# calebhabesh/NM03-Capstone-Project

Hardware: AMD Instinct MI355X
Metric: DICOM slices/sec through full pipeline (T1+C cohort) at 1/2/4/8 MI355X (higher is better)
Workload: dtype fp32

## Files before the change

include/nm03/cohort.h:

```cpp
#pragma once

#include <cstdint>
#include <memory>
#include <string>
#include <vector>

namespace nm03::cohort {

int extract_file_number(const std::string& filename);

std::string default_data_root();
std::string with_slash(const std::string& p);
std::string cohort_dir(const std::string& data_root);
std::string test_slice_path(const std::string& data_root);

std::vector<std::string> find_patient_dirs(const std::string& cohort_root);

struct Series {
  std::string series_dir;
  std::vector<std::string> files;
};
Series list_patient_series(const std::string& cohort_root, const std::string& patient_id);

void setup_output_dir(const std::string& dir);
void setup_output_dirs(const std::vector<std::string>& dirs, int threads);
void make_dirs(const std::string& dir);

class OutputReaper {
 public:
  explicit OutputReaper(int threads = 4);
  ~OutputReaper();
  OutputReaper(const OutputReaper&) = delete;
  OutputReaper& operator=(const OutputReaper&) = delete;
  void wipe(const std::string& dir);
  void wipe(const std::vector<std::string>& dirs);
  void drain();
  int64_t files_reaped() const;

  struct Impl;

 private:
  std::unique_ptr<Impl> impl_;
};

std::string stem(const std::string& path);
std::string filename(const std::string& path);

}
```

include/nm03/dicom.h:

```cpp
#pragma once

#include <cstdint>
#include <memory>
#include <string>
#include <vector>

#include "nm03/common.h"

namespace nm03::dicom {

enum class Syntax : uint8_t {
  kImplicitLE,
  kExplicitLE,
  kExplicitBE,
  kDeflatedLE,
  kRleLossless,
  kJpegLossless,
  kJpegBaseline,
  kJpegExtended,
};

const char* syntax_name(Syntax s);

struct Header {
// ... 10 lines not shown
  double slice_thickness = 0;
  double spacing_between_slices = 0;
  std::string photometric, transfer_syntax, sop_instance_uid, series_uid, patient_id, modality;
  Syntax syntax = Syntax::kExplicitLE;
  size_t pixel_offset = 0;
  size_t pixel_length = 0;
  bool invert = false;
  std::shared_ptr<const std::vector<uint8_t>> decoded;
  size_t frame_bytes() const { return (size_t)rows * cols * (bits_allocated / 8); }
  bool native_le() const { return decoded || syntax != Syntax::kExplicitBE; }
  const uint8_t* pixel_base(const uint8_t* file) const { return decoded ? decoded->data() : file; }
};

Header parse(const uint8_t* data, size_t size);

Header parse_prefix(const uint8_t* data, size_t avail, size_t size);

void copy_pixels16(const Header& h, const uint8_t* data, size_t size, uint16_t* dst, int frame = 0);

int select_frame(const Header& h, int policy);

void invert_samples(uint16_t* px, size_t n, int bits);

std::vector<uint8_t> read_file(const std::string& path);
size_t read_file_into(const std::string& path, std::vector<uint8_t>& buf);

enum class ReadMode { kDirect, kStaged, kMapped };

class SliceFile {
 public:
  explicit SliceFile(const std::string& path, ReadMode mode = ReadMode::kDirect, size_t prefix = 16384);
  SliceFile(int dirfd, const char* name, const std::string& path, ReadMode mode = ReadMode::kDirect,
            size_t prefix = 16384);
  ~SliceFile();
  SliceFile(const SliceFile&) = delete;
  SliceFile& operator=(const SliceFile&) = delete;
  size_t size() const { return size_; }
  void map_at(void* addr, size_t cap) {
    map_at_ = addr;
    map_cap_ = cap;
  }
  const Header& header(std::vector<uint8_t>& buf);
  void pixels16(uint16_t* dst, int frame = 0);
  bool direct() const { return !whole_; }
  const uint16_t* staged_samples(int frame = 0) const;

 private:
  void pread_all(void* dst, size_t n, size_t off);
  void stat_size();
  bool size_known_ = false;
  const uint8_t* data() const { return map_ ? map_ : buf_->data(); }
  std::string path_;
  const uint8_t* map_ = nullptr;
  bool own_map_ = true;
  void* map_at_ = nullptr;
  size_t map_cap_ = 0;
  int fd_ = -1;
  size_t size_ = 0;
  ReadMode mode_ = ReadMode::kDirect;
  size_t prefix_ = 16384;
  size_t have_ = 0;
  Header h_;
  bool whole_ = true;
  std::vector<uint8_t>* buf_ = nullptr;
};

void stream_copy(void* dst, const void* src, size_t n);
void stream_copy_unfenced(void* dst, const void* src, size_t n);

struct WriteSpec {
  int rows = 256, cols = 256;
  PixelType type = kU16;
  int bits_stored = 16;
  const uint16_t* pixels = nullptr;
  bool write_rescale = false;
  float slope = 1.f, intercept = 0.f;
  float spacing_x = 1.f, spacing_y = 1.f;
  double slice_thickness = 1.0;
  double spacing_between_slices = 0;
  int instance_number = 1;
  double position[3] = {0, 0, 0};
  bool write_position = true;
  std::string patient_id = "PGBM-000";
  std::string study_uid = "1.2.826.0.1.3680043.10.1", series_uid = "1.2.826.0.1.3680043.10.2",
              sop_uid = "1.2.826.0.1.3680043.10.3";
// ... 13 lines not shown
```

include/nm03/jpeg.h:

```cpp
#pragma once

#include <atomic>
#include <cstdint>
#include <string>
#include <vector>

#include "nm03/jpeg_common.h"

namespace nm03::jpeg {

struct Tables {
  int quality = 75;
  uint16_t qluma[64];
  uint16_t qchroma[64];
  int32_t div_luma[64];
  int32_t div_chroma[64];
};

Tables make_tables(int quality);

std::vector<uint8_t> make_header(int width, int height, const Tables& t, Sampling s = kSampling420);

std::vector<uint8_t> encode_gray(const uint8_t* gray, int width, int height, int stride, int quality,
                                 Sampling s = kSampling420);

std::vector<uint8_t> encode_scan_gray(const uint8_t* gray, int width, int height, int stride, const Tables& t,
                                      Sampling s = kSampling420);

std::vector<uint8_t> encode_rgb(const uint8_t* rgb, int width, int height, int stride, int quality,
                                Sampling s = kSampling420);
std::vector<uint8_t> encode_scan_rgb(const uint8_t* rgb, int width, int height, int stride, const Tables& t,
                                     Sampling s = kSampling420);

void write_jpeg_file(const std::string& path, const std::vector<uint8_t>& header, const uint8_t* scan,
                     size_t scan_len);
void write_jpeg_at(int dirfd, const std::string& dir, const std::string& name, const std::vector<uint8_t>& header,
                   const uint8_t* scan, size_t scan_len,
                   std::atomic<uint8_t>* creating = nullptr);
void write_bytes_at(int dirfd, const std::string& dir, const std::string& name, const void* data, size_t len,
                    std::atomic<uint8_t>* creating = nullptr);

}
```

src/io/cohort.cpp:

```cpp
#include "nm03/cohort.h"

#include <dirent.h>
#include <fcntl.h>
#include <linux/capability.h>
#include <pthread.h>
#include <signal.h>
#include <sys/stat.h>
#include <sys/syscall.h>
#include <unistd.h>

#include <algorithm>
#include <atomic>
#include <cerrno>
#include <condition_variable>
#include <deque>
#include <mutex>
#include <set>
#include <thread>
#include <cstdlib>
#include <cstring>
#include <filesystem>
#include <stdexcept>
#include <system_error>

// ... 244 lines not shown
void OutputReaper::wipe(const std::string& dir_in) {
  std::string dir = dir_in;
  while (dir.size() > 1 && dir.back() == '/') dir.pop_back();
  const size_t slash = dir.rfind('/');
  const std::string parent = slash == std::string::npos ? "." : slash == 0 ? "/" : dir.substr(0, slash);
  make_dirs(parent);
  impl_->sweep_parent(parent);
  const std::string trash = parent + "/" + kTrashPrefix + std::to_string(::getpid()) + "-" +
                            std::to_string(impl_->seq.fetch_add(1));
  if (::rename(dir.c_str(), trash.c_str()) == 0) {
    impl_->push(trash);
  } else if (errno != ENOENT) {
    setup_output_dir(dir);
    return;
  }
  if (::mkdir(dir.c_str(), 0755) != 0 && errno != EEXIST)
    throw std::runtime_error("Failed to setup output directory: " + dir + " (" + std::strerror(errno) + ")");
}

void OutputReaper::wipe(const std::vector<std::string>& dirs) {
  for (const auto& d : dirs) wipe(d);
}

void OutputReaper::drain() {
  std::unique_lock<std::mutex> g(impl_->m);
  impl_->idle_cv.wait(g, [&] { return impl_->q.empty() && impl_->busy == 0; });
}

int64_t OutputReaper::files_reaped() const { return impl_->files.load(); }

std::string stem(const std::string& path) { return fs::path(path).stem().string(); }
std::string filename(const std::string& path) { return fs::path(path).filename().string(); }

}
```

src/io/dicom.cpp:

```cpp
#include "nm03/dicom.h"
#include "nm03/jpeg_dct.h"
#include "nm03/jpeg_lossless.h"

#include <fcntl.h>
#include <immintrin.h>
#include <sys/mman.h>
#include <sys/stat.h>
#include <unistd.h>
#include <zlib.h>

#include <algorithm>
#include <cerrno>
#include <cstdio>
#include <cstdlib>
#include <cstring>
#include <fstream>

namespace nm03::dicom {
namespace {

constexpr uint32_t kUndefined = 0xFFFFFFFFu;

struct Cursor {
  const uint8_t* d;
// ... 518 lines not shown
    std::memcpy(dst, src, n * 2);
  }
  if (h.invert) invert_samples(dst, n, h.bits_stored);
}

size_t read_file_into(const std::string& path, std::vector<uint8_t>& buf) {
  int fd = ::open(path.c_str(), O_RDONLY | O_CLOEXEC);
  if (fd < 0) throw SliceError("Cannot open file: " + path + " (" + std::strerror(errno) + ")");
  struct stat st;
  if (fstat(fd, &st) != 0) {
    ::close(fd);
    throw SliceError("Cannot stat file: " + path);
  }
  size_t n = (size_t)st.st_size;
  if (buf.size() < n) buf.resize(n);
  size_t got = 0;
  while (got < n) {
    ssize_t r = ::read(fd, buf.data() + got, n - got);
    if (r < 0 && errno == EINTR) continue;
    if (r <= 0) {
      ::close(fd);
      throw SliceError("Read error on file: " + path);
    }
    got += (size_t)r;
  }
  ::close(fd);
  return n;
}

SliceFile::SliceFile(const std::string& path, ReadMode mode, size_t prefix)
    : SliceFile(AT_FDCWD, path.c_str(), path, mode, prefix) {}

SliceFile::SliceFile(int dirfd, const char* name, const std::string& path, ReadMode mode, size_t prefix)
    : path_(path), mode_(mode), prefix_(prefix < 1024 ? 1024 : prefix) {
  fd_ = ::openat(dirfd, name, O_RDONLY | O_CLOEXEC);
  if (fd_ < 0) throw SliceError("Cannot open file: " + path + " (" + std::strerror(errno) + ")");
  if (mode_ == ReadMode::kStaged) return;
  stat_size();
}

void SliceFile::stat_size() {
  struct stat st;
  if (fstat(fd_, &st) != 0) {
    ::close(fd_);
    fd_ = -1;
    throw SliceError("Cannot stat file: " + path_);
  }
  size_ = (size_t)st.st_size;
  size_known_ = true;
}

SliceFile::~SliceFile() {
  if (map_ && own_map_) ::munmap(const_cast<uint8_t*>(map_), size_);
  if (fd_ >= 0) ::close(fd_);
}

void SliceFile::pread_all(void* dst, size_t n, size_t off) {
  size_t got = 0;
  while (got < n) {
    ssize_t r = ::pread(fd_, (uint8_t*)dst + got, n - got, (off_t)(off + got));
    if (r < 0 && errno == EINTR) continue;
    if (r <= 0) throw SliceError("Read error on file: " + path_);
    got += (size_t)r;
  }
}

const Header& SliceFile::header(std::vector<uint8_t>& buf) {
  buf_ = &buf;
  if (mode_ == ReadMode::kStaged && !size_known_) {
    if (buf.size() < (256u << 10)) buf.resize(256u << 10);
    size_t got = 0;
    for (;;) {
      const ssize_t r = ::pread(fd_, buf.data() + got, buf.size() - got, (off_t)got);
      if (r < 0 && errno == EINTR) continue;
      if (r < 0) throw SliceError("Read error on file: " + path_);
      got += (size_t)r;
      if (got < buf.size() || r == 0) break;
      stat_size();
      if (size_ <= got) break;
      buf.resize(size_);
    }
    size_ = got;
    size_known_ = true;
    have_ = size_;
    try {
      h_ = parse(buf.data(), size_);
    } catch (const SliceError&) {
      stat_size();
      if (size_ <= got) throw;
      if (buf.size() < size_) buf.resize(size_);
      pread_all(buf.data() + got, size_ - got, got);
      have_ = size_;
      h_ = parse(buf.data(), size_);
    }
    whole_ = true;
    return h_;
  }
  if (mode_ == ReadMode::kMapped && size_ > 0) {
    const bool fixed = map_at_ && size_ <= map_cap_;
    void* m = ::mmap(fixed ? map_at_ : nullptr, size_, PROT_READ, MAP_PRIVATE | MAP_POPULATE | (fixed ? MAP_FIXED : 0),
                     fd_, 0);
    if (m == MAP_FAILED) throw SliceError("Cannot map file: " + path_);
    own_map_ = !fixed;
    map_ = static_cast<const uint8_t*>(m);
    have_ = size_;
    h_ = parse(map_, size_);
    whole_ = true;
    return h_;
  }
  const size_t pre = mode_ == ReadMode::kStaged ? size_ : std::min(size_, prefix_);
  if (buf.size() < pre) buf.resize(pre);
  pread_all(buf.data(), pre, 0);
  buf_ = &buf;
  have_ = pre;
  if (pre < size_) {
    try {
      h_ = parse_prefix(buf.data(), pre, size_);
      whole_ = false;
      if (h_.bits_allocated == 16 && h_.syntax != Syntax::kExplicitBE && !h_.decoded) return h_;
    } catch (const SliceError&) {
    }
  }
  if (buf.size() < size_) buf.resize(size_);
  if (pre < size_) pread_all(buf.data() + pre, size_ - pre, pre);
  have_ = size_;
  h_ = parse(buf.data(), size_);
  whole_ = true;
  return h_;
}

void SliceFile::pixels16(uint16_t* dst, int frame) {
  if (frame < 0 || frame >= h_.frames) throw SliceError("DICOM frame " + std::to_string(frame) + " out of range");
  const size_t n = (size_t)h_.rows * h_.cols * 2;
  const size_t off = h_.pixel_offset + (size_t)frame * h_.frame_bytes();
  if (whole_) {
// ... 329 lines not shown
```

src/io/jpeg.cpp:

```cpp
#include "nm03/jpeg.h"

#include <fcntl.h>

#include <atomic>
#include <sys/stat.h>
#include <sys/uio.h>
#include <unistd.h>

#include <cerrno>
#include <cstring>
#include <stdexcept>

namespace nm03::jpeg {

Tables make_tables(int quality) {
  Tables t;
  t.quality = quality;
  quality_table(kStdLuma, quality, t.qluma);
  quality_table(kStdChroma, quality, t.qchroma);
  for (int i = 0; i < 64; ++i) {
    t.div_luma[i] = (int32_t)t.qluma[i] * 8;
    t.div_chroma[i] = (int32_t)t.qchroma[i] * 8;
  }
  return t;
// ... 237 lines not shown
          plane_block(py.data(), width, height, width, bx, by, t.div_luma, zz);
        } else {
          std::memset(zz, 0, sizeof(zz));
          zz[0] = (int16_t)last_dc_y;
        }
        encode_block(w, zz, last_dc_y, kHuffDcLuma, kHuffAcLuma);
      }
      plane_block(dcb.data(), cw, ch, cw, mx, my, t.div_chroma, zz);
      encode_block(w, zz, last_dc_cb, kHuffDcChroma, kHuffAcChroma);
      plane_block(dcr.data(), cw, ch, cw, mx, my, t.div_chroma, zz);
      encode_block(w, zz, last_dc_cr, kHuffDcChroma, kHuffAcChroma);
    }
  }
  w.flush();
  return out;
}

std::vector<uint8_t> encode_rgb(const uint8_t* rgb, int width, int height, int stride, int quality, Sampling s) {
  if (s != kSampling420 && s != kSampling444) throw std::invalid_argument("encode_rgb: a colour image needs 4:2:0 or 4:4:4");
  Tables t = make_tables(quality);
  std::vector<uint8_t> f = make_header(width, height, t, s);
  std::vector<uint8_t> sc = encode_scan_rgb(rgb, width, height, stride, t, s);
  f.insert(f.end(), sc.begin(), sc.end());
  f.push_back(0xFF);
  f.push_back(0xD9);
  return f;
}

void write_jpeg_file(const std::string& path, const std::vector<uint8_t>& header, const uint8_t* scan, size_t scan_len) {
  write_jpeg_at(AT_FDCWD, "", path, header, scan, scan_len);
}

namespace {
void write_parts_at(int dirfd, const std::string& dir, const std::string& name, struct iovec* iov, int nparts,
                    std::atomic<uint8_t>* creating);
}

void write_jpeg_at(int dirfd, const std::string& dir, const std::string& name, const std::vector<uint8_t>& header,
                   const uint8_t* scan, size_t scan_len, std::atomic<uint8_t>* creating) {
  static const uint8_t eoi[2] = {0xFF, 0xD9};
  struct iovec iov[3] = {{(void*)header.data(), header.size()}, {(void*)scan, scan_len}, {(void*)eoi, 2}};
  write_parts_at(dirfd, dir, name, iov, 3, creating);
}

void write_bytes_at(int dirfd, const std::string& dir, const std::string& name, const void* data, size_t len,
                    std::atomic<uint8_t>* creating) {
  struct iovec iov[1] = {{(void*)data, len}};
  write_parts_at(dirfd, dir, name, iov, 1, creating);
}

namespace {
void write_parts_at(int dirfd, const std::string& dir, const std::string& name, struct iovec* iov, int nparts,
                    std::atomic<uint8_t>* creating) {
  auto path = [&] { return dir.empty() ? name : dir + "/" + name; };
  int fd = -1;
  bool fresh = false;
  if (creating && creating->load(std::memory_order_relaxed) != 1) {
    fd = ::openat(dirfd, name.c_str(), O_WRONLY | O_CLOEXEC);
    if (fd < 0 && errno == ENOENT) creating->store(1, std::memory_order_relaxed);
  }
  if (fd < 0 && creating) {
    fd = ::openat(dirfd, name.c_str(), O_WRONLY | O_CREAT | O_EXCL | O_CLOEXEC, 0644);
    fresh = fd >= 0;
  }
  if (fd < 0) fd = ::openat(dirfd, name.c_str(), O_WRONLY | O_CREAT | O_CLOEXEC, 0644);
  if (fd < 0) throw std::runtime_error("Cannot create " + path() + ": " + std::strerror(errno));
  size_t total = 0;
  for (int k = 0; k < nparts; ++k) total += iov[k].iov_len;
  size_t done = 0;
  int idx = 0;
  while (done < total) {
    ssize_t w = ::pwritev(fd, iov + idx, nparts - idx, (off_t)done);
    if (w < 0 && errno == EINTR) continue;
    if (w <= 0) {
      ::close(fd);
      throw std::runtime_error("Write failed: " + path());
    }
    done += (size_t)w;
    size_t adv = (size_t)w;
    while (idx < nparts && adv >= iov[idx].iov_len) {
      adv -= iov[idx].iov_len;
      ++idx;
    }
    if (idx < nparts) {
      iov[idx].iov_base = (uint8_t*)iov[idx].iov_base + adv;
      iov[idx].iov_len -= adv;
    }
  }
  const off_t end = fresh ? 0 : ::lseek(fd, 0, SEEK_END);
  if (end > (off_t)total && ftruncate(fd, (off_t)total) != 0) {
    ::close(fd);
    throw std::runtime_error("Truncate failed: " + path());
  }
  ::close(fd);
}
}

}
// ... 1 lines not shown
```

src/python/bindings.cpp:

```cpp
#include <hip/hip_runtime_api.h>
#include <pybind11/functional.h>
#include <pybind11/numpy.h>
#include <pybind11/pybind11.h>
#include <pybind11/stl.h>

#include <sys/mman.h>
#include <unistd.h>

#include <algorithm>
#include <chrono>
#include <cstring>
#include <mutex>
#include <thread>
#include <vector>

#include "nm03/app.h"
#include "nm03/cohort.h"
#include "nm03/comm.h"
#include "nm03/cpu_sampler.h"
#include "nm03/dicom.h"
#include "nm03/engine.h"
#include "nm03/metaimage.h"
#include "nm03/numa.h"
#include "nm03/golden.h"
// ... 978 lines not shown
                                               : std::vector<py::ssize_t>{im.h, im.w};
    py::array a;
    switch (im.type) {
      case mhd::MetType::kUChar: a = py::array_t<uint8_t>(shape); break;
      case mhd::MetType::kUShort: a = py::array_t<uint16_t>(shape); break;
      case mhd::MetType::kShort: a = py::array_t<int16_t>(shape); break;
      case mhd::MetType::kFloat: a = py::array_t<float>(shape); break;
    }
    std::memcpy(a.mutable_data(), im.bytes.data(), im.bytes.size());
    return py::make_tuple(a, py::make_tuple(im.spacing[0], im.spacing[1], im.spacing[2]));
  });
  m.def("numa_node_cpus", &numa::node_cpus);
  m.def("numa_device_node", &numa::device_node, py::arg("device"));
  m.def("device_bus_id", &numa::device_bus_id, py::arg("device"));
  m.def("cpu_budget", &numa::cpu_budget, py::arg("cgroup_root") = "/sys/fs/cgroup");
  m.def("allowed_cpus", &numa::allowed_cpus);
  m.def("format_cpulist", &numa::format_cpulist);
  m.def(
      "rank_partition",
      [](const std::vector<int>& rank_nodes, int local_rank, int budget, int cap, const std::string& sysfs,
         const std::vector<int>& allowed) {
        const numa::Topology t = numa::read_topology(sysfs, allowed);
        const numa::RankCpus r = numa::rank_partition(t, rank_nodes, local_rank, budget, cap);
        py::dict d;
        d["node"] = r.node;
        d["index"] = r.index;
        d["count"] = r.count;
        d["cpus"] = r.cpus;
        d["threads"] = r.threads;
        return d;
      },
      py::arg("rank_nodes"), py::arg("local_rank"), py::arg("budget"), py::arg("cap") = 16,
      py::arg("sysfs") = "/sys", py::arg("allowed") = std::vector<int>{});
  m.def(
      "read_pixels_direct",
      [](const std::string& path, const std::string& mode, size_t prefix, int frame) {
        dicom::SliceFile f(path, mode == "staged" ? dicom::ReadMode::kStaged : dicom::ReadMode::kDirect, prefix);
        std::vector<uint8_t> scratch;
        const dicom::Header& h = f.header(scratch);
        std::vector<uint16_t> px((size_t)h.rows * h.cols + 1);
        uint16_t* dst = px.data() + 1;
        f.pixels16(dst, frame);
        std::vector<uint16_t> out(dst, dst + (size_t)h.rows * h.cols);
        const uint16_t* ss = f.staged_samples(frame);
        py::object staged = py::none();
        if (ss) staged = to_np<uint16_t>(std::vector<uint16_t>(ss, ss + (size_t)h.rows * h.cols), {h.rows, h.cols});
        return py::make_tuple(to_np<uint16_t>(out, {h.rows, h.cols}), f.direct(), staged);
      },
      py::arg("path"), py::arg("mode") = "direct", py::arg("prefix") = 16384, py::arg("frame") = 0);
  m.def(
      "read_slice",
      [](const std::string& path, int min_dim, int frame) {
        golden::SliceInput s = golden::load_slice(path, min_dim, frame);
        py::dict meta;
        meta["type"] = s.type == kI16 ? "i16" : "u16";
        meta["stored_bits"] = s.stored_bits;
        meta["slope"] = s.slope;
        meta["intercept"] = s.intercept;
        meta["spacing_x"] = s.spacing_x;
        meta["spacing_y"] = s.spacing_y;
        return py::make_tuple(to_np<uint16_t>(s.raw, {s.h, s.w}), meta);
      },
      py::arg("path"), py::arg("min_dim") = 0, py::arg("frame") = -1);

  m.def("extract_file_number", &cohort::extract_file_number);
  m.def("auto_gpus", &app::auto_gpus, py::arg("slices"), py::arg("visible"));
// ... 678 lines not shown
    py::array_t<int32_t> codes((py::ssize_t)st.size());
    auto c = codes.mutable_unchecked<1>();
    py::dict msgs;
    for (size_t i = 0; i < st.size(); ++i) {
      c((py::ssize_t)i) = st[i].code;
      if (st[i].code != kSliceOk) msgs[py::int_(i)] = st[i].message;
    }
    return py::make_tuple(codes, msgs, times_dict(t));
  };
  py::class_<Engine>(m, "Engine")
      .def(py::init<const EngineConfig&>())
      .def(
          "run",
          [times_dict](Engine& e, const std::vector<std::pair<std::string, std::string>>& items) {
            std::vector<WorkItem> wi;
            for (auto& p : items) wi.push_back({p.first, p.second});
            StageTimes t;
            std::vector<SliceStatus> st;
            {
              py::gil_scoped_release nogil;
              st = e.run(wi, &t);
            }
            std::vector<std::pair<int, std::string>> out;
            for (auto& s : st) out.push_back({s.code, s.message});
            return py::make_tuple(out, times_dict(t));
          })
      .def(
          "run_list",
          [compact](Engine& e, const WorkList& wl, int batch_cap) {
            StageTimes t;
            std::vector<SliceStatus> st;
            {
              py::gil_scoped_release nogil;
              st = e.run(*wl.items, &t, {}, batch_cap);
            }
            return compact(st, t);
          },
          py::arg("work"), py::arg("batch_cap") = 0)
      .def(
          "submit",
          [](Engine& e, const WorkList& wl, int batch_cap) {
            py::gil_scoped_release nogil;
            return Ticket{e.submit(wl.items, {}, batch_cap)};
          },
          py::arg("work"), py::arg("batch_cap") = 0)
      .def(
          "wait",
          [compact](Engine& e, const Ticket& t) {
            StageTimes tm;
            std::vector<SliceStatus> st;
            {
              py::gil_scoped_release nogil;
              st = e.wait(t.t, &tm);
            }
            return compact(st, tm);
          })
      .def("run_single",
           [](Engine& e, py::array_t<uint16_t, py::array::c_style | py::array::forcecast> raw, const std::string& type,
              int stored_bits, float slope, float intercept, float sx, float sy) {
             golden::SliceInput s = slice_from(raw, type, stored_bits, slope, intercept, sx, sy);
             SingleResult r;
             {
               py::gil_scoped_release nogil;
               r = e.run_single(s);
             }
             py::dict d;
             d["median_keys"] = to_np<uint16_t>(r.median_keys, {r.h, r.w});
// ... 1637 lines not shown
```

src/runtime/engine.cpp:

```cpp
#include "nm03/engine.h"

#include <hip/hip_runtime_api.h>
#include <fcntl.h>
#include <linux/capability.h>
#include <signal.h>
#include <sys/mman.h>
#include <sys/prctl.h>
#include <sys/resource.h>
#include <sys/syscall.h>
#include <unistd.h>

#include <algorithm>
#include <ctime>
#include <atomic>
#include <array>
#include <chrono>
#include <condition_variable>
#include <cstdlib>
#include <cstring>
#include <deque>
#include <unordered_map>
#include <mutex>
#include <tuple>
#include <thread>
// ... 99 lines not shown
  bool arena = false;
  size_t out_bytes = 0;
  uint8_t* d_rgb = nullptr;
  JpegWork ov_jw;
  uint8_t* h_ov_out = nullptr;
  uint8_t* d_ov_out = nullptr;
  int32_t* h_ov_sizes = nullptr;
  int32_t* d_ov_sizes = nullptr;
  JpegDesc* d_ov_jd = nullptr;
  uint32_t* d_ms_scratch = nullptr;
  SliceMeasure* h_measure = nullptr;
  SliceMeasure* d_measure = nullptr;
  SliceDiameters* h_diam = nullptr;
  SliceDiameters* d_diam = nullptr;
  IntensityStats* h_intensity = nullptr;
  IntensityStats* d_intensity = nullptr;
  uint8_t* h_texture = nullptr;
  uint8_t* d_texture = nullptr;
};

static void make_fd_table_private() {
#ifndef CLOSE_RANGE_UNSHARE
#define CLOSE_RANGE_UNSHARE (1U << 1)
#endif
  (void)::syscall(SYS_close_range, 3u, ~0u, CLOSE_RANGE_UNSHARE);
}

static void make_cred_private() {
  __user_cap_header_struct h{_LINUX_CAPABILITY_VERSION_3, 0};
  __user_cap_data_struct c[2]{};
  if (::syscall(SYS_capget, &h, c) == 0) (void)::syscall(SYS_capset, &h, c);
}

struct IoDirs {
  size_t ndirs = 0;
  std::unique_ptr<std::atomic<uint8_t>[]> creating;
  std::vector<int32_t> out_dir;
  explicit IoDirs(const std::vector<WorkItem>& items) {
    std::unordered_map<std::string, int32_t> idx;
    out_dir.resize(items.size());
    for (size_t i = 0; i < items.size(); ++i) {
      auto it = idx.emplace(items[i].out_dir, (int32_t)idx.size()).first;
      out_dir[i] = it->second;
    }
    ndirs = idx.size();
    creating.reset(new std::atomic<uint8_t>[std::max<size_t>(ndirs, 1)]);
    for (size_t k = 0; k < ndirs; ++k) creating[k].store(0, std::memory_order_relaxed);
  }
  IoDirs(const IoDirs&) = delete;
  IoDirs& operator=(const IoDirs&) = delete;
};

void hip_free_all(Slot& s) {
  if (s.host_only) {
    if (s.h_blob) munmap(s.h_blob, s.blob_bytes);
    if (s.h_out) munmap(s.h_out, s.out_bytes);
    delete[] s.h_sizes;
    return;
  }
  if (!s.arena) {
    if (s.h_blob) (void)hipHostFree(s.h_blob);
    if (s.h_out) (void)hipHostFree(s.h_out);
    if (s.h_sizes) (void)hipHostFree(s.h_sizes);
  }
  if (s.h_single) (void)hipHostFree(s.h_single);
  if (s.h_ov_out) (void)hipHostFree(s.h_ov_out);
  if (s.h_ov_sizes) (void)hipHostFree(s.h_ov_sizes);
  if (s.h_measure) (void)hipHostFree(s.h_measure);
  if (s.h_diam) (void)hipHostFree(s.h_diam);
  if (s.h_intensity) (void)hipHostFree(s.h_intensity);
  if (s.h_texture) (void)hipHostFree(s.h_texture);
  if (s.d_ms_scratch) (void)hipFree(s.d_ms_scratch);
  for (void* p : {(void*)s.d_rgb, (void*)s.ov_jw.look, (void*)s.ov_jw.ticket, (void*)s.ov_jw.spill, (void*)s.d_ov_jd})
    if (p) (void)hipFree(p);
  for (void* p : {(void*)s.d_blob, (void*)s.d_raw_x, (void*)s.d_med, (void*)s.d_tile_mm, (void*)s.d_f32, (void*)s.d_bits, (void*)s.d_srg_scratch, (void*)s.d_canvas,
                  (void*)s.jw.look, (void*)s.jw.ticket, (void*)s.jw.spill})
    if (p) (void)hipFree(p);
  if (s.ev0) (void)hipEventDestroy(s.ev0);
// ... 538 lines not shown
    if (nslices <= 16) {
      const double until = t_enq + 1e-3;
      for (;;) {
        const hipError_t e = hipEventQuery(ev);
        if (e == hipSuccess) return;
        if (e != hipErrorNotReady) check_hip(e, "batch sync");
        if (now_s() > until) break;
        for (int k = 0; k < 32; ++k) __builtin_ia32_pause();
      }
    }
    const double scale = (double)std::max(1, nslices);
    const double target = 0.8 * s.batch_ema_s * scale;
    for (;;) {
      const hipError_t e = hipEventQuery(ev);
      if (e == hipSuccess) break;
      if (e != hipErrorNotReady) check_hip(e, "batch sync");
      const double ahead = target - (now_s() - t_enq);
      if (ahead > 100e-6)
        std::this_thread::sleep_for(std::chrono::duration<double>(std::min(ahead, 250e-6)));
      else
        std::this_thread::sleep_for(std::chrono::microseconds(20));
    }
    const double took = (now_s() - t_enq) / scale;
    s.batch_ema_s = s.batch_ema_s > 0 ? 0.75 * s.batch_ema_s + 0.25 * took : took;
  }

  void load_into(Slot& s, int i, size_t item, const std::string& path, SliceStatus& st, std::atomic<int64_t>& load_ns,
                 std::atomic<int64_t>& bytes_in) {
    thread_local std::vector<uint8_t> buf;
    TraceRange tr("nm03.load");
    const double t0 = now_s();
    try {
      if (fault_plan().corrupt_dicom == (int64_t)item) throw SliceError("injected fault: corrupt DICOM data");
      dicom::SliceFile file(AT_FDCWD, path.c_str(), path, dicom::ReadMode::kStaged);
      const dicom::Header& h = file.header(buf);
      const int frame = dicom::select_frame(h, cfg.pipe.frame);
      const size_t n = file.size();
      const int md = cfg.pipe.min_dim;
      if (md > 0 && (h.cols < md || h.rows < md)) {
        st.code = kSliceTooSmall;
        st.message = "Image dimensions too small: " + std::to_string(h.cols) + "x" + std::to_string(h.rows);
      } else if (h.cols > cfg.max_dim || h.rows > cfg.max_dim) {
        st.code = kSliceLoadError;
        st.message = "Image dimensions " + std::to_string(h.cols) + "x" + std::to_string(h.rows) +
                     " exceed the engine limit " + std::to_string(cfg.max_dim);
      } else {
        const size_t npix = (size_t)h.rows * h.cols;
        const uint16_t* samples = pack12_ ? file.staged_samples(frame) : nullptr;
        const size_t plen = align_up(npix / 4 * 3, 8), ulen = align_up(npix, 8);
        const bool packable = samples && pack12::available() && (npix & 15) == 0;
        const size_t cap = s.cap_pixels + s.hole_slack;
        size_t idx = 0, off = 0;
        bool packed = false, reserved = false, credit = false;
        auto reserve = [&](size_t len) {
          uint64_t w = s.alloc_word.load(std::memory_order_relaxed);
          for (;;) {
            const size_t used = (size_t)(w & Slot::kUsedMask), n = (size_t)(w >> Slot::kAllocShift);
            if (used + len > cap) throw SliceError("batch pixel capacity exceeded");
            if (n >= s.max_allocs) throw SliceError("batch allocation table full");
            const uint64_t nw = ((uint64_t)(n + 1) << Slot::kAllocShift) | (uint64_t)(used + len);
            if (s.alloc_word.compare_exchange_weak(w, nw, std::memory_order_acq_rel, std::memory_order_relaxed)) {
              idx = n;
              off = used;
              break;
            }
          }
          s.allocs[idx].off = off;
// ... 34 lines not shown
            if (packed) {
              pack12::pack_stream(samples, npix, reinterpret_cast<uint8_t*>(dst));
            } else {
              file.pixels16(dst, frame);
            }
          }
        } catch (...) {
          if (reserved) s.allocs[idx].done.store(true, std::memory_order_release);
          throw;
        }
        s.allocs[idx].done.store(true, std::memory_order_release);
        LoadedSlice& L = s.loaded[i];
        L.w = h.cols;
        L.h = h.rows;
        L.type = h.type == kU8 ? kU16 : h.type;
        L.stored_bits = (uint8_t)(h.type == kU8 ? 8 : h.bits_stored);
        L.slope = cfg.pipe.apply_rescale ? h.slope : 1.f;
        L.intercept = cfg.pipe.apply_rescale ? h.intercept : 0.f;
        L.sx = h.spacing_x;
        L.sy = h.spacing_y;
        L.blob_off = (uint32_t)off;
        L.packed = packed;
        L.ok = true;
        st.code = kSliceOk;
        bytes_in += (int64_t)n;
      }
    } catch (const std::exception& e) {
      st.code = kSliceLoadError;
      st.message = e.what();
    }
    load_ns += (int64_t)((now_s() - t0) * 1e9);
  }

  bool outputs_exist(const WorkItem& w) const {
    const std::string base = cohort::with_slash(w.out_dir) + cohort::stem(w.path);
    return access((base + "_original.jpg").c_str(), F_OK) == 0 && access((base + "_processed.jpg").c_str(), F_OK) == 0 &&
           (!overlay_ || access((base + "_overlay.jpg").c_str(), F_OK) == 0) &&
           (!measure_ || access((base + "_measure.json").c_str(), F_OK) == 0);
  }

  static inline thread_local std::vector<Seed> seeds_cache_;
  static inline thread_local int seeds_w_ = 0, seeds_h_ = 0;
  void build_and_run(Slot& s, int mode, StageTimes* acc, BatchMark* mark = nullptr) {
    const int nl = (int)s.live.size();
    uint8_t* hb = s.h_blob;
    auto* stats = reinterpret_cast<SliceStats*>(hb + s.off_stats);
    auto* desc = reinterpret_cast<SliceDesc*>(hb + s.off_desc);
    auto* medt = reinterpret_cast<TileDesc*>(hb + s.off_medt);
    auto* shpt = reinterpret_cast<TileDesc*>(hb + s.off_shpt);
    auto* seeds = reinterpret_cast<SeedXY*>(hb + s.off_seeds);
    auto* rd = reinterpret_cast<RenderDesc*>(hb + s.off_render);
    auto* jd = reinterpret_cast<JpegDesc*>(hb + s.off_jpeg);
    int nmed = 0, nshp = 0, nseed = 0, ncanv = 0;
    s.any_canvas = false;
    uint32_t mask_off = 0;
    s.max_w = s.max_h = 0;
    const int cw = cfg.render.out_width, ch = cfg.render.out_height;
    const uint32_t canvas_bytes = (uint32_t)(cw * ch);
    const uint8_t fill = opacity_u8(cfg.render.label_opacity), bval = opacity_u8(cfg.render.border_opacity);
    uint32_t xoff = 0;
    for (int c = 0; c < nl; ++c) {
      const LoadedSlice& L = s.loaded[s.live[c]];
      stats[c] = SliceStats{0xFFFFFFFFu, 0u, 0xFFFFFFFFu, 0u};
      SliceDesc& d = desc[c];
      std::memset(&d, 0, sizeof(d));
      const uint32_t raw_off = xoff;
      xoff += (uint32_t)align_up((size_t)L.w * L.h, 8);
      d.raw_off = raw_off;
      d.blob_off = L.blob_off;
      d.flags = L.packed ? kSliceFlagPacked12 : 0;
      d.w = (uint16_t)L.w;
// ... 233 lines not shown
    if (intensity_)
      return measure::to_json(m, s.h_intensity[c], L.w, L.h, L.sx, L.sy, L.slope, L.intercept, cfg.pipe.apply_rescale,
                              cfg.pipe.measure_connectivity);
    return measure::to_json(m, L.w, L.h, L.sx, L.sy, L.slope, L.intercept, cfg.pipe.apply_rescale,
                            cfg.pipe.measure_connectivity);
  }

  static int small_batch_spin(size_t count) { return count <= 16 ? 200 : 0; }
  void process_batch(Slot& s, const std::vector<WorkItem>& items, const IoDirs& dirs, size_t batch, uint64_t prio,
                     size_t first, size_t count, std::vector<SliceStatus>& status, StageTimes& acc,
                     std::mutex& acc_m, const std::function<void(size_t)>& on_start, BatchMark* mark = nullptr) {
    if (mark) mark->claim = now_s();
    s.loaded.assign(count, LoadedSlice{});
    if (!s.allocs) {
      s.max_allocs = 2 * (size_t)s.cap_slices;
      s.allocs.reset(new Slot::Alloc[s.max_allocs]);
    }
    for (size_t k = 0; k < s.max_allocs; ++k) s.allocs[k].done.store(false, std::memory_order_relaxed);
    s.alloc_word.store(0, std::memory_order_relaxed);
    s.hole_credit.store(s.hole_slack, std::memory_order_relaxed);
    s.uploaded = 0;
    s.upload_started = false;
    s.loads_finished.store(0, std::memory_order_relaxed);
    s.wake_at.store(0, std::memory_order_relaxed);
    s.progress_quiet.store(false, std::memory_order_relaxed);
    std::atomic<int64_t> load_ns{0}, bytes_in{0}, write_ns{0}, bytes_out{0}, load_cpu_ns{0}, write_cpu_ns{0};
    std::string upload_error;
    {
      TaskGroup tg(*pool);
      tg.for_each(
          count,
          [&](size_t i) {
            if (on_start) on_start(first + i);
            if (cfg.resume && outputs_exist(items[first + i])) {
              status[first + i] = SliceStatus{kSliceOk, "resumed: outputs already present"};
            } else {
              load_into(s, (int)i, first + i, items[first + i].path, status[first + i], load_ns, bytes_in);
            }
            if (upload_chunk_) {
              const size_t lf = s.loads_finished.fetch_add(1, std::memory_order_seq_cst) + 1;
              if (!s.progress_quiet.load(std::memory_order_relaxed) &&
                  (lf >= s.wake_at.load(std::memory_order_seq_cst) || lf == count) &&
                  s.prog_waiting.load(std::memory_order_seq_cst)) {
                { std::lock_guard<std::mutex> g(s.prog_m); }
                s.prog_cv.notify_one();
              }
            }
          },
          2 * prio, &load_cpu_ns);
      if (upload_chunk_) {
        try {
          upload_progress(s, count);
        } catch (const std::exception& e) {
          upload_error = e.what();
        }
      }
      tg.wait(small_batch_spin(count));
    }
    if (mark) mark->loaded = now_s();
    s.live.clear();
    for (size_t i = 0; i < count; ++i)
      if (s.loaded[i].ok) s.live.push_back((int)i);
    if (s.live.empty() && s.upload_started) check_hip(hipStreamSynchronize(s.up), "upload drain");
    StageTimes local;
    int64_t fallbacks = 0;
    if (!s.live.empty()) {
      try {
// ... 24 lines not shown
      std::vector<char> use_ofb(ofb.size(), 0);
      for (size_t c = 0; c < ofb.size(); ++c) {
        try {
          use_ofb[c] = !overlay_segment(s, (int)c, ofb[c], &fallbacks);
        } catch (const std::exception& e) {
          status[first + s.live[c]] = SliceStatus{kSliceExportError, e.what()};
        }
      }
      std::vector<int> order(s.live.size());
      if (dirs.ndirs > 1) {
        std::vector<std::pair<int32_t, std::vector<int>>> groups;
        for (size_t c = 0; c < s.live.size(); ++c) {
          const int32_t d = dirs.out_dir[first + s.live[c]];
          auto it = std::find_if(groups.rbegin(), groups.rend(), [&](const auto& g) { return g.first == d; });
          if (it == groups.rend()) {
            groups.push_back({d, {}});
            it = groups.rbegin();
          }
          it->second.push_back((int)c);
        }
        size_t o = 0;
        for (size_t r = 0; o < order.size(); ++r)
          for (auto& g : groups)
            if (r < g.second.size()) order[o++] = g.second[r];
      } else {
        for (size_t c = 0; c < order.size(); ++c) order[c] = (int)c;
      }
      bool creates = false;
      for (int c : s.live) {
        const size_t item = first + (size_t)c;
        std::atomic<uint8_t>& st = dirs.creating[dirs.out_dir[item]];
        uint8_t v = st.load(std::memory_order_relaxed);
        if (v == 0) {
          const std::string f = cohort::with_slash(items[item].out_dir) + cohort::stem(items[item].path) + "_original.jpg";
          const uint8_t probe = ::access(f.c_str(), F_OK) == 0 ? 2 : (errno == ENOENT ? 1 : 2);
          st.compare_exchange_strong(v, probe, std::memory_order_relaxed);
          v = st.load(std::memory_order_relaxed);
        }
        creates = creates || v == 1;
      }
      TaskGroup tg(*pool);
      tg.for_each(
          s.live.size(),
          [&](size_t oc) {
            const size_t c = (size_t)order[oc];
            const size_t item = first + s.live[c];
            if (status[item].code != kSliceOk) return;
            const double t0 = now_s();
            TraceRange tr("nm03.export");
            try {
              if (fault_plan().fail_write == (int64_t)item) throw std::runtime_error("injected fault: export failure");
              const std::string base = cohort::with_slash(items[item].out_dir) + cohort::stem(items[item].path);
              for (int k = 0; k < 2; ++k) {
                const int cv = 2 * (int)c + k;
                const std::string name = base + (k == 0 ? "_original.jpg" : "_processed.jpg");
                const uint8_t* seg = use_fb[cv] ? fb[cv].data() : jpeg_bytes(s, cv);
                const size_t len = use_fb[cv] ? fb[cv].size() : (size_t)s.h_sizes[cv];
                jpeg::write_jpeg_at(AT_FDCWD, std::string(), name, jpeg_header, seg, len,
                                    &dirs.creating[dirs.out_dir[item]]);
                bytes_out += (int64_t)(jpeg_header.size() + len + 2);
              }
              if (overlay_) {
                const uint8_t* seg = use_ofb[c] ? ofb[c].data() : s.h_ov_out + c * (size_t)ov_cap_;
                const size_t len = use_ofb[c] ? ofb[c].size() : (size_t)s.h_ov_sizes[c];
                jpeg::write_jpeg_at(AT_FDCWD, std::string(), base + "_overlay.jpg", jpeg_header, seg, len,
                                    &dirs.creating[dirs.out_dir[item]]);
                bytes_out += (int64_t)(jpeg_header.size() + len + 2);
              }
              if (measure_) {
                const std::string js = measure_text(s, (int)c);
                jpeg::write_bytes_at(AT_FDCWD, std::string(), base + "_measure.json", js.data(), js.size(),
                                     &dirs.creating[dirs.out_dir[item]]);
                bytes_out += (int64_t)js.size();
              }
            } catch (const std::exception& e) {
              status[item] = SliceStatus{kSliceExportError, std::string("Error in export stage: ") + e.what()};
            }
            write_ns += (int64_t)((now_s() - t0) * 1e9);
          },
          2 * prio + 1, &write_cpu_ns, creates ? cfg.create_writers : 0);
      tg.wait(small_batch_spin(count));
    }
    if (mark) mark->end = now_s();
    std::lock_guard<std::mutex> g(acc_m);
    acc.load_s += load_ns.load() * 1e-9;
    acc.write_s += write_ns.load() * 1e-9;
    acc.load_cpu_s += load_cpu_ns.load() * 1e-9;
    acc.write_cpu_s += write_cpu_ns.load() * 1e-9;
    acc.h2d_s += local.h2d_s;
    acc.kernels_s += local.kernels_s;
    acc.bytes_in += bytes_in.load();
    acc.bytes_out += bytes_out.load();
    acc.jpeg_fallbacks += fallbacks;
    acc.batches += 1;
  }

  static std::vector<std::pair<size_t, size_t>> plan_batches(size_t n, size_t B) {
    std::vector<std::pair<size_t, size_t>> out;
    if (n == 0 || B == 0) return out;
    const size_t k = (n + B - 1) / B, q = n / k, rem = n % k;
    size_t first = 0;
    for (size_t b = 0; b < k; ++b) {
      const size_t len = q + (b < rem ? 1 : 0);
      out.push_back({first, len});
// ... 110 lines not shown
      }
      {
        std::unique_lock<std::mutex> g(job_m);
        job_cv.wait(g, [&] { return quit || !queue.empty(); });
        if (queue.empty()) return;
        j = queue.front();
        b = j->next++;
        if (j->next == j->batches.size()) queue.pop_front();
        queued_jobs_.store(queue.size(), std::memory_order_release);
      }
      const int64_t c0 = thread_cpu_ns();
      try {
        const auto [first, count] = j->batches[b];
        BatchMark* mk = j->marks.empty() ? nullptr : &j->marks[b];
        if (mk) {
          mk->slot = (int)slot_index;
          mk->first = first;
          mk->count = count;
        }
        process_batch(*s, *j->items, *j->dirs, b, j->seq0 + b, first, count, j->status, j->acc, j->acc_m,
                      j->on_start, mk);
      } catch (...) {
        std::lock_guard<std::mutex> g(j->err_m);
        if (!j->err) j->err = std::current_exception();
      }
      {
        std::lock_guard<std::mutex> g(j->acc_m);
        j->acc.slot_cpu_s += (thread_cpu_ns() - c0) * 1e-9;
      }
      if (j->remaining.fetch_sub(1) == 1) finish(*j);
    }
  }

  std::shared_ptr<Job> submit(std::shared_ptr<const std::vector<WorkItem>> items, std::function<void(size_t)> on_start,
                              int batch_cap = 0) {
    auto j = std::make_shared<Job>();
    j->t0 = now_s();
    j->items = std::move(items);
    j->dirs = std::make_unique<IoDirs>(*j->items);
    j->on_start = std::move(on_start);
    j->status.resize(j->items->size());
    const size_t B = batch_cap > 0 ? std::min<size_t>((size_t)batch_cap, (size_t)cfg.batch_size) : (size_t)cfg.batch_size;
    j->batches = plan_batches(j->items->size(), B);
    j->remaining = j->batches.size();
    if (batch_trace()) j->marks.resize(j->batches.size());
    {
      std::lock_guard<std::mutex> g(job_m);
      j->seq0 = seq_next;
      seq_next += j->batches.size();
      ++inflight;
      if (!j->batches.empty()) queue.push_back(j);
      queued_jobs_.store(queue.size(), std::memory_order_release);
    }
    if (j->batches.empty())
      finish(*j);
    else
      job_cv.notify_all();
    return j;
  }

  std::vector<SliceStatus> wait(const std::shared_ptr<Job>& j, StageTimes* times) {
    {
      std::unique_lock<std::mutex> g(job_m);
      done_cv.wait(g, [&] { return j->done; });
    }
    if (j->err) std::rethrow_exception(j->err);
    if (times) *times = j->acc;
    return j->status;
  }

  std::vector<SliceStatus> run(const std::vector<WorkItem>& items, StageTimes* times,
                               const std::function<void(size_t)>& on_start, int batch_cap = 0) {
// ... 174 lines not shown
```

Measured before the change: 477,300.

## Precompute output file names in an arena and cache them per work list

Output JPEG names (`_original`/`_processed`) are now built once per work item into a contiguous char arena (`OutputNames`) instead of being rebuilt on every export and resume probe with `with_slash` plus a `std::filesystem` stem. The arena is held in a `WorkNames` object that is cached across submits, keyed by a weak pointer to the item list. The Python binding now submits the shared item list so repeated runs can hit this cache. `SliceFile` can borrow the path as a `const char*`, and the JPEG writers take C-string names, removing per-slice string allocations on the load and write paths. The cost is extra memory for the arena, a mutex-guarded cache lookup per submit, and thread_local scratch strings for the overlay and measure names.

```diff
diff --git a/include/nm03/cohort.h b/include/nm03/cohort.h
--- a/include/nm03/cohort.h
+++ b/include/nm03/cohort.h
@@ -46,4 +46,22 @@
 std::string stem(const std::string& path);
 std::string filename(const std::string& path);
 
+class OutputNames {
+ public:
+  void reserve(size_t items, size_t bytes = 0);
+  void add(const std::string& path, const std::string& out_dir);
+  size_t size() const { return off_.size(); }
+  const char* original(size_t i) const { return arena_.data() + off_[i].original; }
+  const char* processed(size_t i) const { return arena_.data() + off_[i].processed; }
+  size_t base_len(size_t i) const { return off_[i].base_len; }
+  std::string base(size_t i) const { return std::string(original(i), base_len(i)); }
+
+ private:
+  struct Off {
+    uint32_t original, processed, base_len;
+  };
+  std::vector<char> arena_;
+  std::vector<Off> off_;
+};
+
 }
diff --git a/include/nm03/dicom.h b/include/nm03/dicom.h
--- a/include/nm03/dicom.h
+++ b/include/nm03/dicom.h
@@ -66,6 +66,10 @@
   explicit SliceFile(const std::string& path, ReadMode mode = ReadMode::kDirect, size_t prefix = 16384);
   SliceFile(int dirfd, const char* name, const std::string& path, ReadMode mode = ReadMode::kDirect,
             size_t prefix = 16384);
+  struct BorrowedPath {
+    const char* c_str;
+  };
+  explicit SliceFile(BorrowedPath path, ReadMode mode = ReadMode::kDirect, size_t prefix = 16384);
   ~SliceFile();
   SliceFile(const SliceFile&) = delete;
   SliceFile& operator=(const SliceFile&) = delete;
@@ -82,9 +86,11 @@
  private:
   void pread_all(void* dst, size_t n, size_t off);
   void stat_size();
+  void open_at(int dirfd, const char* name);
   bool size_known_ = false;
   const uint8_t* data() const { return map_ ? map_ : buf_->data(); }
-  std::string path_;
+  std::string owned_path_;
+  const char* path_ = nullptr;
   const uint8_t* map_ = nullptr;
   bool own_map_ = true;
   void* map_at_ = nullptr;
diff --git a/include/nm03/jpeg.h b/include/nm03/jpeg.h
--- a/include/nm03/jpeg.h
+++ b/include/nm03/jpeg.h
@@ -39,5 +39,9 @@
                    std::atomic<uint8_t>* creating = nullptr);
 void write_bytes_at(int dirfd, const std::string& dir, const std::string& name, const void* data, size_t len,
                     std::atomic<uint8_t>* creating = nullptr);
+void write_jpeg_at(int dirfd, const char* dir, const char* name, const std::vector<uint8_t>& header,
+                   const uint8_t* scan, size_t scan_len, std::atomic<uint8_t>* creating = nullptr);
+void write_bytes_at(int dirfd, const char* dir, const char* name, const void* data, size_t len,
+                    std::atomic<uint8_t>* creating = nullptr);
 
 }
diff --git a/src/io/cohort.cpp b/src/io/cohort.cpp
--- a/src/io/cohort.cpp
+++ b/src/io/cohort.cpp
@@ -300,4 +300,23 @@
 std::string stem(const std::string& path) { return fs::path(path).stem().string(); }
 std::string filename(const std::string& path) { return fs::path(path).filename().string(); }
 
-}
+void OutputNames::reserve(size_t items, size_t bytes) {
+  off_.reserve(items);
+  if (bytes) arena_.reserve(bytes);
+}
+
+void OutputNames::add(const std::string& path, const std::string& out_dir) {
+  static const char* const kSuffix[2] = {"_original.jpg", "_processed.jpg"};
+  const std::string base = with_slash(out_dir) + stem(path);
+  if (arena_.size() + 2 * (base.size() + 16) > UINT32_MAX) throw std::length_error("OutputNames: more than 4 GiB of file names");
+  Off o{};
+  o.base_len = (uint32_t)base.size();
+  for (int k = 0; k < 2; ++k) {
+    (k == 0 ? o.original : o.processed) = (uint32_t)arena_.size();
+    arena_.insert(arena_.end(), base.begin(), base.end());
+    arena_.insert(arena_.end(), kSuffix[k], kSuffix[k] + std::strlen(kSuffix[k]) + 1);
+  }
+  off_.push_back(o);
+}
+
+}
diff --git a/src/io/dicom.cpp b/src/io/dicom.cpp
--- a/src/io/dicom.cpp
+++ b/src/io/dicom.cpp
@@ -574,9 +574,18 @@
     : SliceFile(AT_FDCWD, path.c_str(), path, mode, prefix) {}
 
 SliceFile::SliceFile(int dirfd, const char* name, const std::string& path, ReadMode mode, size_t prefix)
-    : path_(path), mode_(mode), prefix_(prefix < 1024 ? 1024 : prefix) {
+    : owned_path_(path), path_(owned_path_.c_str()), mode_(mode), prefix_(prefix < 1024 ? 1024 : prefix) {
+  open_at(dirfd, name);
+}
+
+SliceFile::SliceFile(BorrowedPath path, ReadMode mode, size_t prefix)
+    : path_(path.c_str), mode_(mode), prefix_(prefix < 1024 ? 1024 : prefix) {
+  open_at(AT_FDCWD, path_);
+}
+
+void SliceFile::open_at(int dirfd, const char* name) {
   fd_ = ::openat(dirfd, name, O_RDONLY | O_CLOEXEC);
-  if (fd_ < 0) throw SliceError("Cannot open file: " + path + " (" + std::strerror(errno) + ")");
+  if (fd_ < 0) throw SliceError(std::string("Cannot open file: ") + path_ + " (" + std::strerror(errno) + ")");
   if (mode_ == ReadMode::kStaged) return;
   stat_size();
 }
@@ -586,7 +595,7 @@
   if (fstat(fd_, &st) != 0) {
     ::close(fd_);
     fd_ = -1;
-    throw SliceError("Cannot stat file: " + path_);
+    throw SliceError(std::string("Cannot stat file: ") + path_);
   }
   size_ = (size_t)st.st_size;
   size_known_ = true;
@@ -602,7 +611,7 @@
   while (got < n) {
     ssize_t r = ::pread(fd_, (uint8_t*)dst + got, n - got, (off_t)(off + got));
     if (r < 0 && errno == EINTR) continue;
-    if (r <= 0) throw SliceError("Read error on file: " + path_);
+    if (r <= 0) throw SliceError(std::string("Read error on file: ") + path_);
     got += (size_t)r;
   }
 }
@@ -615,7 +624,7 @@
     for (;;) {
       const ssize_t r = ::pread(fd_, buf.data() + got, buf.size() - got, (off_t)got);
       if (r < 0 && errno == EINTR) continue;
-      if (r < 0) throw SliceError("Read error on file: " + path_);
+      if (r < 0) throw SliceError(std::string("Read error on file: ") + path_);
       got += (size_t)r;
       if (got < buf.size() || r == 0) break;
       stat_size();
@@ -642,7 +651,7 @@
     const bool fixed = map_at_ && size_ <= map_cap_;
     void* m = ::mmap(fixed ? map_at_ : nullptr, size_, PROT_READ, MAP_PRIVATE | MAP_POPULATE | (fixed ? MAP_FIXED : 0),
                      fd_, 0);
-    if (m == MAP_FAILED) throw SliceError("Cannot map file: " + path_);
+    if (m == MAP_FAILED) throw SliceError(std::string("Cannot map file: ") + path_);
     own_map_ = !fixed;
     map_ = static_cast<const uint8_t*>(m);
     have_ = size_;
diff --git a/src/io/jpeg.cpp b/src/io/jpeg.cpp
--- a/src/io/jpeg.cpp
+++ b/src/io/jpeg.cpp
@@ -293,38 +293,48 @@
 }
 
 namespace {
-void write_parts_at(int dirfd, const std::string& dir, const std::string& name, struct iovec* iov, int nparts,
+void write_parts_at(int dirfd, const char* dir, const char* name, struct iovec* iov, int nparts,
                     std::atomic<uint8_t>* creating);
 }
 
-void write_jpeg_at(int dirfd, const std::string& dir, const std::string& name, const std::vector<uint8_t>& header,
+void write_jpeg_at(int dirfd, const char* dir, const char* name, const std::vector<uint8_t>& header,
                    const uint8_t* scan, size_t scan_len, std::atomic<uint8_t>* creating) {
   static const uint8_t eoi[2] = {0xFF, 0xD9};
   struct iovec iov[3] = {{(void*)header.data(), header.size()}, {(void*)scan, scan_len}, {(void*)eoi, 2}};
   write_parts_at(dirfd, dir, name, iov, 3, creating);
 }
 
-void write_bytes_at(int dirfd, const std::string& dir, const std::string& name, const void* data, size_t len,
+void write_jpeg_at(int dirfd, const std::string& dir, const std::string& name, const std::vector<uint8_t>& header,
+                   const uint8_t* scan, size_t scan_len, std::atomic<uint8_t>* creating) {
+  write_jpeg_at(dirfd, dir.c_str(), name.c_str(), header, scan, scan_len, creating);
+}
+
+void write_bytes_at(int dirfd, const char* dir, const char* name, const void* data, size_t len,
                     std::atomic<uint8_t>* creating) {
   struct iovec iov[1] = {{(void*)data, len}};
   write_parts_at(dirfd, dir, name, iov, 1, creating);
 }
 
+void write_bytes_at(int dirfd, const std::string& dir, const std::string& name, const void* data, size_t len,
+                    std::atomic<uint8_t>* creating) {
+  write_bytes_at(dirfd, dir.c_str(), name.c_str(), data, len, creating);
+}
+
 namespace {
-void write_parts_at(int dirfd, const std::string& dir, const std::string& name, struct iovec* iov, int nparts,
+void write_parts_at(int dirfd, const char* dir, const char* name, struct iovec* iov, int nparts,
                     std::atomic<uint8_t>* creating) {
-  auto path = [&] { return dir.empty() ? name : dir + "/" + name; };
+  auto path = [&] { return !dir || !*dir ? std::string(name) : std::string(dir) + "/" + name; };
   int fd = -1;
   bool fresh = false;
   if (creating && creating->load(std::memory_order_relaxed) != 1) {
-    fd = ::openat(dirfd, name.c_str(), O_WRONLY | O_CLOEXEC);
+    fd = ::openat(dirfd, name, O_WRONLY | O_CLOEXEC);
     if (fd < 0 && errno == ENOENT) creating->store(1, std::memory_order_relaxed);
   }
   if (fd < 0 && creating) {
-    fd = ::openat(dirfd, name.c_str(), O_WRONLY | O_CREAT | O_EXCL | O_CLOEXEC, 0644);
+    fd = ::openat(dirfd, name, O_WRONLY | O_CREAT | O_EXCL | O_CLOEXEC, 0644);
     fresh = fd >= 0;
   }
-  if (fd < 0) fd = ::openat(dirfd, name.c_str(), O_WRONLY | O_CREAT | O_CLOEXEC, 0644);
+  if (fd < 0) fd = ::openat(dirfd, name, O_WRONLY | O_CREAT | O_CLOEXEC, 0644);
   if (fd < 0) throw std::runtime_error("Cannot create " + path() + ": " + std::strerror(errno));
   size_t total = 0;
   for (int k = 0; k < nparts; ++k) total += iov[k].iov_len;
diff --git a/src/python/bindings.cpp b/src/python/bindings.cpp
--- a/src/python/bindings.cpp
+++ b/src/python/bindings.cpp
@@ -1034,6 +1034,14 @@
       },
       py::arg("rank_nodes"), py::arg("local_rank"), py::arg("budget"), py::arg("cap") = 16,
       py::arg("sysfs") = "/sys", py::arg("allowed") = std::vector<int>{});
+  m.def("output_names", [](const std::vector<std::pair<std::string, std::string>>& items) {
+    cohort::OutputNames n;
+    n.reserve(items.size());
+    for (const auto& p : items) n.add(p.first, p.second);
+    std::vector<std::tuple<std::string, std::string, std::string>> out;
+    for (size_t i = 0; i < n.size(); ++i) out.emplace_back(n.original(i), n.processed(i), n.base(i));
+    return out;
+  });
   m.def(
       "read_pixels_direct",
       [](const std::string& path, const std::string& mode, size_t prefix, int frame) {
@@ -1778,7 +1786,7 @@
             std::vector<SliceStatus> st;
             {
               py::gil_scoped_release nogil;
-              st = e.run(*wl.items, &t, {}, batch_cap);
+              st = e.wait(e.submit(wl.items, {}, batch_cap), &t);
             }
             return compact(st, t);
           },
diff --git a/src/runtime/engine.cpp b/src/runtime/engine.cpp
--- a/src/runtime/engine.cpp
+++ b/src/runtime/engine.cpp
@@ -155,18 +155,31 @@
   if (::syscall(SYS_capget, &h, c) == 0) (void)::syscall(SYS_capset, &h, c);
 }
 
-struct IoDirs {
+struct WorkNames {
   size_t ndirs = 0;
-  std::unique_ptr<std::atomic<uint8_t>[]> creating;
   std::vector<int32_t> out_dir;
-  explicit IoDirs(const std::vector<WorkItem>& items) {
+  cohort::OutputNames files;
+  explicit WorkNames(const std::vector<WorkItem>& items) {
     std::unordered_map<std::string, int32_t> idx;
     out_dir.resize(items.size());
+    files.reserve(items.size());
     for (size_t i = 0; i < items.size(); ++i) {
       auto it = idx.emplace(items[i].out_dir, (int32_t)idx.size()).first;
       out_dir[i] = it->second;
+      files.add(items[i].path, items[i].out_dir);
     }
     ndirs = idx.size();
+  }
+};
+
+struct IoDirs {
+  std::shared_ptr<const WorkNames> names;
+  const size_t ndirs;
+  std::unique_ptr<std::atomic<uint8_t>[]> creating;
+  const std::vector<int32_t>& out_dir;
+  const cohort::OutputNames& files;
+  explicit IoDirs(std::shared_ptr<const WorkNames> n)
+      : names(std::move(n)), ndirs(names->ndirs), out_dir(names->out_dir), files(names->files) {
     creating.reset(new std::atomic<uint8_t>[std::max<size_t>(ndirs, 1)]);
     for (size_t k = 0; k < ndirs; ++k) creating[k].store(0, std::memory_order_relaxed);
   }
@@ -771,7 +784,7 @@
     const double t0 = now_s();
     try {
       if (fault_plan().corrupt_dicom == (int64_t)item) throw SliceError("injected fault: corrupt DICOM data");
-      dicom::SliceFile file(AT_FDCWD, path.c_str(), path, dicom::ReadMode::kStaged);
+      dicom::SliceFile file(dicom::SliceFile::BorrowedPath{path.c_str()}, dicom::ReadMode::kStaged);
       const dicom::Header& h = file.header(buf);
       const int frame = dicom::select_frame(h, cfg.pipe.frame);
       const size_t n = file.size();
@@ -872,11 +885,16 @@
     load_ns += (int64_t)((now_s() - t0) * 1e9);
   }
 
-  bool outputs_exist(const WorkItem& w) const {
-    const std::string base = cohort::with_slash(w.out_dir) + cohort::stem(w.path);
-    return access((base + "_original.jpg").c_str(), F_OK) == 0 && access((base + "_processed.jpg").c_str(), F_OK) == 0 &&
-           (!overlay_ || access((base + "_overlay.jpg").c_str(), F_OK) == 0) &&
-           (!measure_ || access((base + "_measure.json").c_str(), F_OK) == 0);
+  bool outputs_exist(const IoDirs& dirs, size_t item) const {
+    return access(dirs.files.original(item), F_OK) == 0 && access(dirs.files.processed(item), F_OK) == 0 &&
+           (!overlay_ || access(side_name(dirs, item, "_overlay.jpg"), F_OK) == 0) &&
+           (!measure_ || access(side_name(dirs, item, "_measure.json"), F_OK) == 0);
+  }
+  static const char* side_name(const IoDirs& dirs, size_t item, const char* suffix) {
+    thread_local std::string name;
+    name.assign(dirs.files.original(item), dirs.files.base_len(item));
+    name += suffix;
+    return name.c_str();
   }
 
   static inline thread_local std::vector<Seed> seeds_cache_;
@@ -1176,7 +1194,7 @@
           count,
           [&](size_t i) {
             if (on_start) on_start(first + i);
-            if (cfg.resume && outputs_exist(items[first + i])) {
+            if (cfg.resume && outputs_exist(dirs, first + i)) {
               status[first + i] = SliceStatus{kSliceOk, "resumed: outputs already present"};
             } else {
               load_into(s, (int)i, first + i, items[first + i].path, status[first + i], load_ns, bytes_in);
@@ -1267,8 +1285,7 @@
         std::atomic<uint8_t>& st = dirs.creating[dirs.out_dir[item]];
         uint8_t v = st.load(std::memory_order_relaxed);
         if (v == 0) {
-          const std::string f = cohort::with_slash(items[item].out_dir) + cohort::stem(items[item].path) + "_original.jpg";
-          const uint8_t probe = ::access(f.c_str(), F_OK) == 0 ? 2 : (errno == ENOENT ? 1 : 2);
+          const uint8_t probe = ::access(dirs.files.original(item), F_OK) == 0 ? 2 : (errno == ENOENT ? 1 : 2);
           st.compare_exchange_strong(v, probe, std::memory_order_relaxed);
           v = st.load(std::memory_order_relaxed);
         }
@@ -1285,26 +1302,24 @@
             TraceRange tr("nm03.export");
             try {
               if (fault_plan().fail_write == (int64_t)item) throw std::runtime_error("injected fault: export failure");
-              const std::string base = cohort::with_slash(items[item].out_dir) + cohort::stem(items[item].path);
               for (int k = 0; k < 2; ++k) {
                 const int cv = 2 * (int)c + k;
-                const std::string name = base + (k == 0 ? "_original.jpg" : "_processed.jpg");
+                const char* name = k == 0 ? dirs.files.original(item) : dirs.files.processed(item);
                 const uint8_t* seg = use_fb[cv] ? fb[cv].data() : jpeg_bytes(s, cv);
                 const size_t len = use_fb[cv] ? fb[cv].size() : (size_t)s.h_sizes[cv];
-                jpeg::write_jpeg_at(AT_FDCWD, std::string(), name, jpeg_header, seg, len,
-                                    &dirs.creating[dirs.out_dir[item]]);
+                jpeg::write_jpeg_at(AT_FDCWD, nullptr, name, jpeg_header, seg, len, &dirs.creating[dirs.out_dir[item]]);
                 bytes_out += (int64_t)(jpeg_header.size() + len + 2);
               }
               if (overlay_) {
                 const uint8_t* seg = use_ofb[c] ? ofb[c].data() : s.h_ov_out + c * (size_t)ov_cap_;
                 const size_t len = use_ofb[c] ? ofb[c].size() : (size_t)s.h_ov_sizes[c];
-                jpeg::write_jpeg_at(AT_FDCWD, std::string(), base + "_overlay.jpg", jpeg_header, seg, len,
+                jpeg::write_jpeg_at(AT_FDCWD, nullptr, side_name(dirs, item, "_overlay.jpg"), jpeg_header, seg, len,
                                     &dirs.creating[dirs.out_dir[item]]);
                 bytes_out += (int64_t)(jpeg_header.size() + len + 2);
               }
               if (measure_) {
                 const std::string js = measure_text(s, (int)c);
-                jpeg::write_bytes_at(AT_FDCWD, std::string(), base + "_measure.json", js.data(), js.size(),
+                jpeg::write_bytes_at(AT_FDCWD, nullptr, side_name(dirs, item, "_measure.json"), js.data(), js.size(),
                                      &dirs.creating[dirs.out_dir[item]]);
                 bytes_out += (int64_t)js.size();
               }
@@ -1481,12 +1496,39 @@
     }
   }
 
+  struct NamesEntry {
+    std::weak_ptr<const std::vector<WorkItem>> list;
+    std::shared_ptr<const WorkNames> names;
+  };
+  static constexpr size_t kNamesCached = 8;
+  std::mutex names_m_;
+  std::deque<NamesEntry> names_cache_;
+  std::shared_ptr<const WorkNames> names_for(const std::shared_ptr<const std::vector<WorkItem>>& items) {
+    {
+      std::lock_guard<std::mutex> g(names_m_);
+      for (auto it = names_cache_.begin(); it != names_cache_.end();) {
+        if (it->list.expired()) {
+          it = names_cache_.erase(it);
+          continue;
+        }
+        if (!it->list.owner_before(items) && !items.owner_before(it->list) && it->names->out_dir.size() == items->size())
+          return it->names;
+        ++it;
+      }
+    }
+    auto names = std::make_shared<const WorkNames>(*items);
+    std::lock_guard<std::mutex> g(names_m_);
+    if (names_cache_.size() >= kNamesCached) names_cache_.pop_front();
+    names_cache_.push_back({items, names});
+    return names;
+  }
+
   std::shared_ptr<Job> submit(std::shared_ptr<const std::vector<WorkItem>> items, std::function<void(size_t)> on_start,
                               int batch_cap = 0) {
     auto j = std::make_shared<Job>();
     j->t0 = now_s();
     j->items = std::move(items);
-    j->dirs = std::make_unique<IoDirs>(*j->items);
+    j->dirs = std::make_unique<IoDirs>(names_for(j->items));
     j->on_start = std::move(on_start);
     j->status.resize(j->items->size());
     const size_t B = batch_cap > 0 ? std::min<size_t>((size_t)batch_cap, (size_t)cfg.batch_size) : (size_t)cfg.batch_size;
```

Measured after the change: 476,100. About the same (-0.3%).
